# jaak-s/BayesianDataFusion.jl

Measured on AMD Instinct MI355X. Metric: Gibbs sweeps/sec (both entities) + test RMSE, MovieLens-1M D=32, higher is better.
Workload: dtype f64; 1 GPU; BPMF MovieLens-1M 6040x3952, 500209 training ratings (500000 held out), D=32, alpha=1.5, step = rows of both entities + hyperpriors + test prediction update (one native call); BEFORE the --warmup steps the engine's set-up runs 60 ms of full iterations whose results are discarded (device_warmup_ms); num_latent=32, burnin=5, psamples=1985, parallelism=1 GPU

## Files before the change

bayesiandatafusion.jl_amd/csrc/k_rows_col.hip:

```cpp
#include "rows.h"
#include "dpp_rows32.h"
#include <algorithm>

#ifndef BDF_COL_WAVES
#define BDF_COL_WAVES 2
#endif
#define COL_PSZ 800

#ifdef BDF_K1_STAMPS
#define CSTAMP_DECL unsigned long long st_t = __builtin_amdgcn_s_memtime(), st_acc = 0, st_mid = 0, st_prior = 0, st_fin = 0, st_rng = 0, st_steps = 0, st_rounds = 0, st_parts = 0, st_fins = 0, st_folds = 0; const unsigned long long st_begin = st_t
#define CSTAMP(x) do { const unsigned long long now_ = __builtin_amdgcn_s_memtime(); x += now_ - st_t; st_t = now_; } while (0)
#else
#define CSTAMP_DECL do { } while (0)
#define CSTAMP(x) do { } while (0)
#endif

namespace {

template <int DR, int K>
__device__ __forceinline__ void col_obs(double (&A0)[33], double (&A1)[33], double v0, double v1, double r)
{
    col_rank1<DR, 0>(A0, A1, v0, v1);
    fm1_run<K>(A0[32], r, v0);
    fm1_run<K>(A1[32], r, v1);
}

__device__ __forceinline__ double col_ld(__amdgpu_buffer_rsrc_t rs, uint32_t off)
{
    typedef unsigned u2v __attribute__((ext_vector_type(2)));
    const u2v x = __builtin_amdgcn_raw_buffer_load_b64(rs, (int)off, 0, 0);
    return __hiloint2double((int)x.y, (int)x.x);
}

template <bool FULL, int K0>
__device__ __forceinline__ void col_gather4(double (&b)[4][2], __amdgpu_buffer_rsrc_t rs, uint32_t idw, uint32_t rowb, uint32_t eo, bool ok1)
{
#pragma unroll
    for (int q = 0; q < 4; q++) {
        uint32_t id;
        if (q == 0) id = row_bcast_u32<K0>(idw); else if (q == 1) id = row_bcast_u32<K0 + 1>(idw);
        else if (q == 2) id = row_bcast_u32<K0 + 2>(idw); else id = row_bcast_u32<K0 + 3>(idw);
        if constexpr (FULL) {
            const uint32_t base = id + eo;
            b[q][1] = col_ld(rs, base);
            b[q][0] = col_ld(rs, base + 128u);
        } else {
            const uint32_t base = id + eo;
            b[q][0] = col_ld(rs, base);
            b[q][1] = col_ld(rs, ok1 ? base - 128u : 0xffffffffu);
        }
    }
}
template <int DR, int K0>
__device__ __forceinline__ void col_compute4(double (&A0)[33], double (&A1)[33], const double (&b)[4][2], double r)
{
    col_obs<DR, K0>(A0, A1, b[0][0], b[0][1], r);
    col_obs<DR, K0 + 1>(A0, A1, b[1][0], b[1][1], r);
    col_obs<DR, K0 + 2>(A0, A1, b[2][0], b[2][1], r);
    col_obs<DR, K0 + 3>(A0, A1, b[3][0], b[3][1], r);
}

template <int X>
__device__ __forceinline__ void col_fold(double (&A0)[33], double (&A1)[33], double m)
{
#pragma unroll
    for (int i = 0; i < 33; i++) A0[i] = fma(__shfl_xor(A0[i], X), m, A0[i]);
#pragma unroll
    for (int i = 16; i < 33; i++) A1[i] = fma(__shfl_xor(A1[i], X), m, A1[i]);
}

template <int E0, int E1, bool ADD>
__device__ __forceinline__ void col_slot_load(double (&A0)[33], double (&A1)[33], const double *src, double m)
{
#pragma unroll
    for (int e = E0; e < E1; e++) {
        const double v = src[e * 16];
        double &d = e < 33 ? A0[e] : A1[e - 17];
        if (ADD) d = fma(v, m, d); else d = v * m;
    }
}

__device__ __forceinline__ void col_prior_dma(const double *image, unsigned lds_dst, int lane)
{
    const void *sbase = (const void *)(((uint64_t)(uint32_t)__builtin_amdgcn_readfirstlane((int)((uint64_t)image >> 32)) << 32) |
                                       (uint32_t)__builtin_amdgcn_readfirstlane((int)(uint32_t)(uint64_t)image));
#pragma unroll
    for (int k = 0; k < 6; k++) {
        const unsigned voff = (unsigned)k * 1024u + (unsigned)lane * 16u;
        unsigned keep;
        asm volatile("s_mov_b32 %0, m0\n\ts_mov_b32 m0, %2\n\ts_nop 0\n\tglobal_load_lds_dwordx4 %1, %3 sc1\n\ts_mov_b32 m0, %0"
                     : "=&s"(keep) : "v"(voff), "s"(lds_dst + (unsigned)k * 1024u), "s"(sbase) : "memory");
    }
}
template <int S, int I, int DR>
__device__ __forceinline__ void col_prior_lds(double (&A)[33], const double *img, double alpha, int j)
{
    if constexpr (I < DR) {
        A[I] = fma(alpha, A[I], img[sys_off<S, I>(j)]);
        col_prior_lds<S, I + 1, DR>(A, img, alpha, j);
    }
}

template <int DR, bool FULL>
__global__ __launch_bounds__(64, BDF_COL_WAVES) void k_rows_col(SampleArgs a_in, ColPlanDev p_in, uint32_t fac_bytes)
{
    __shared__ __attribute__((aligned(16))) double lds[4 * 272 + 768];
    const int w = blockIdx.x;
    if (w >= p_in.n_waves) return;
    const int r_end = p_in.wave_round[w + 1];
    if (a_in.span && threadIdx.x == 0) atomicMin(a_in.span + 2 * (w & 63), (unsigned long long)__builtin_amdgcn_s_memrealtime());
    CSTAMP_DECL;
#pragma nounroll
    for (int rd = p_in.wave_round[w]; rd < r_end; rd++) {
    int zero = 0, lane = threadIdx.x;
    asm volatile("" : "+s"(zero), "+v"(lane));
    const SampleArgs &a = (&a_in)[zero];
    const ColPlanDev &p = (&p_in)[zero];
    const int j = lane & 15, g = lane >> 4;
    const TermDev &T = a.t[0];
    const int D = FULL ? 32 : a.D;
    const int ec0 = D - 1 - j, ec1 = D - 17 - j;
    const int n0 = ec0, n1 = ec1 >= 0 ? ec1 : 0;
    const bool ok1 = ec1 >= 0;
    const uint32_t rowb = (uint32_t)D * 8u;
    const uint32_t eo = FULL ? (uint32_t)ec1 * 8u : (uint32_t)ec0 * 8u;
    const __amdgpu_buffer_rsrc_t rs = __builtin_amdgcn_make_buffer_rsrc((void *)T.fac[0], 0, (int)fac_bytes, 0x00020000);
    const bool coded = T.packed != nullptr;
    const double mean = T.mean;
    {
        const ColJob jb = p.jobs[(int64_t)rd * 4 + g];
        const bool live = jb.row >= 0;
        const int n = live ? jb.count : 0;
        const unsigned lds_img = (unsigned)__builtin_amdgcn_readfirstlane((int)(unsigned)(size_t)(__attribute__((address_space(3))) double *)(lds + 4 * 272));
        bool have_prior = true;
        if (a.ready) have_prior = __builtin_amdgcn_readfirstlane((int)((int32_t)(__hip_atomic_load(a.ready, __ATOMIC_RELAXED, __HIP_MEMORY_SCOPE_AGENT) - a.ready_want) >= 0)) != 0;
        if (have_prior) col_prior_dma(a.prior_c, lds_img, lane);
        double A0[33], A1[33];
#pragma unroll
        for (int i = 0; i < 33; i++) { A0[i] = 0.0; A1[i] = 0.0; }
        int nmax = n;
        nmax = max(nmax, __shfl_xor(nmax, 16));
        nmax = max(nmax, __shfl_xor(nmax, 32));
        nmax = __builtin_amdgcn_readfirstlane(nmax);
        if (nmax > 0) {
            const uint32_t *packed = coded ? T.packed + jb.q_begin : nullptr;
            const int32_t *colidx = T.colidx + jb.q_begin;
            const double *vals = T.vals + jb.q_begin;
            const double *table = T.table;
#define COL_CHUNK(c0, IDW, R)                                                                     \
            {                                                                                     \
                const int o_ = (c0) + j;                                                          \
                IDW = 0xffffffu; R = 0.0;                                                         \
                if (o_ < n) {                                                                     \
                    if (coded) { const uint32_t pw_ = packed[o_]; IDW = pw_; R = table[pw_ >> 24] - mean; } \
                    else { IDW = (uint32_t)colidx[o_]; R = vals[o_] - mean; }                     \
                }                                                                                 \
                IDW = __umul24(IDW, rowb);       \
            }
            uint32_t idw_c, idw_n;
            double r_c, r_n;
            COL_CHUNK(0, idw_c, r_c)
            double ba[4][2], bb[4][2];
            col_gather4<FULL, 0>(ba, rs, idw_c, rowb, eo, ok1);
            for (int c0 = 0;; c0 += 16) {
                COL_CHUNK(c0 + 16, idw_n, r_n)
                col_gather4<FULL, 4>(bb, rs, idw_c, rowb, eo, ok1);
                __builtin_amdgcn_sched_barrier(0);
                col_compute4<DR, 0>(A0, A1, ba, r_c);
                if (c0 + 4 >= nmax) break;
                col_gather4<FULL, 8>(ba, rs, idw_c, rowb, eo, ok1);
                __builtin_amdgcn_sched_barrier(0);
                col_compute4<DR, 4>(A0, A1, bb, r_c);
                if (c0 + 8 >= nmax) break;
                col_gather4<FULL, 12>(bb, rs, idw_c, rowb, eo, ok1);
                __builtin_amdgcn_sched_barrier(0);
                col_compute4<DR, 8>(A0, A1, ba, r_c);
                if (c0 + 12 >= nmax) break;
                col_gather4<FULL, 0>(ba, rs, idw_n, rowb, eo, ok1);
                __builtin_amdgcn_sched_barrier(0);
                col_compute4<DR, 12>(A0, A1, bb, r_c);
                if (c0 + 16 >= nmax) break;
                idw_c = idw_n; r_c = r_n;
            }
#undef COL_CHUNK
        }
#ifdef BDF_K1_STAMPS
        asm volatile("s_nop 0" :: "v"(A0[0]), "v"(A0[32]), "v"(A1[31]));
        st_steps += (unsigned long long)nmax; st_rounds++;
#endif
        CSTAMP(st_acc);
        const unsigned fl = (unsigned)jb.flags;
        if (__builtin_amdgcn_readfirstlane((int)(__ballot((fl & COLF_PAIR) != 0) != 0ull))) {
#ifdef BDF_K1_STAMPS
            st_folds++;
#endif
            col_fold<16>(A0, A1, (fl & COLF_PAIR) ? 1.0 : 0.0);
            if (__builtin_amdgcn_readfirstlane((int)(__ballot((fl & COLF_QUAD) != 0) != 0ull)))
                col_fold<32>(A0, A1, (fl & COLF_QUAD) ? 1.0 : 0.0);
        }
        if (__builtin_amdgcn_readfirstlane((int)(fl & COLF_MULTI))) {
            const int srow = __builtin_amdgcn_readfirstlane(jb.srow);
            double *dst = p.partials + (int64_t)__builtin_amdgcn_readfirstlane(jb.slot) * COL_PSZ + j;
            if (g == 0) {
#pragma unroll
                for (int e = 0; e < 33; e++) __hip_atomic_store(dst + e * 16, A0[e], __ATOMIC_RELAXED, __HIP_MEMORY_SCOPE_AGENT);
#pragma unroll
                for (int e = 33; e < 50; e++) __hip_atomic_store(dst + e * 16, A1[e - 17], __ATOMIC_RELAXED, __HIP_MEMORY_SCOPE_AGENT);
            }
            const ColSplit sr = p.rows[srow];
            asm volatile("s_waitcnt vmcnt(0)" ::: "memory");
            int old = 0;
            if (lane == 0) old = __hip_atomic_fetch_add(p.arrived + srow, 1, __ATOMIC_RELAXED, __HIP_MEMORY_SCOPE_AGENT);
            old = __builtin_amdgcn_readfirstlane(old);
#ifdef BDF_K1_STAMPS
            st_parts++;
            if (old == sr.n_slots - 1) st_fins++;
#endif
            if (old != sr.n_slots - 1) { CSTAMP(st_mid); continue; }
            __builtin_amdgcn_fence(__ATOMIC_ACQUIRE, "agent");
            asm volatile("s_waitcnt vmcnt(0)" ::: "memory");
            if (lane == 0) p.arrived[srow] = 0;
            const double *src = p.partials + (int64_t)sr.slot_begin * COL_PSZ + j;
            col_slot_load<0, 50, false>(A0, A1, src + (int64_t)(g < sr.n_slots ? g : 0) * COL_PSZ, g < sr.n_slots ? 1.0 : 0.0);
            for (int s0 = 4; s0 < sr.n_slots; s0 += 4) {
                const bool on = s0 + g < sr.n_slots;
                const double *sp = src + (int64_t)(on ? s0 + g : 0) * COL_PSZ;
                const double m = on ? 1.0 : 0.0;
                col_slot_load<0, 16, true>(A0, A1, sp, m);
                asm volatile("" ::: "memory");
                col_slot_load<16, 33, true>(A0, A1, sp, m);
                asm volatile("" ::: "memory");
                col_slot_load<33, 50, true>(A0, A1, sp, m);
                asm volatile("" ::: "memory");
            }
            col_fold<16>(A0, A1, 1.0);
            col_fold<32>(A0, A1, 1.0);
        }
        CSTAMP(st_mid);
        double z0 = 0.0, z1 = 0.0;
        {
            double ze = 0.0, zo = 0.0;
            if (live && 2 * j < D) bdf_normal_pair(a.seed, a.sweep, BDF_P_ROW, a.entity_tag, (uint64_t)(uint32_t)jb.orig, (uint32_t)j, ze, zo);
            const int base = lane & 48;
            const double ze0 = __shfl(ze, base + (n0 >> 1)), zo0 = __shfl(zo, base + (n0 >> 1));
            const double ze1 = __shfl(ze, base + (n1 >> 1)), zo1 = __shfl(zo, base + (n1 >> 1));
            z0 = (n0 & 1) ? zo0 : ze0;
            z1 = ok1 ? ((n1 & 1) ? zo1 : ze1) : 0.0;
        }
        asm volatile("" ::: "memory");
        CSTAMP(st_rng);
        {
            double *tl = lds + g * 272;
#pragma unroll
            for (int r = 0; r < 16; r++) tl[r * 17 + j] = A0[16 + r];
            wave_sync();
#pragma unroll
            for (int i = 0; i < 16; i++) A1[i] = tl[j * 17 + i];
            wave_sync();
        }
        CSTAMP(st_mid);
        const double alpha = term_alpha(T);
        if (!have_prior) {
            int spins = 0;
            while ((int32_t)(__hip_atomic_load(a.ready, __ATOMIC_RELAXED, __HIP_MEMORY_SCOPE_AGENT) - a.ready_want) < 0) {
                __builtin_amdgcn_s_sleep(16);
                if (++spins > (1 << 22)) { if (lane == 0) atomicOr_system(a.flag, 16); break; }
            }
            col_prior_dma(a.prior_c, lds_img, lane);
        }
        {
            const double *pb = a.prior_b + (a.mu_is_matrix && live ? (int64_t)jb.row * D : 0);
            const double b0 = __hip_atomic_load(pb + n0, __ATOMIC_RELAXED, __HIP_MEMORY_SCOPE_AGENT);
            const double b1 = __hip_atomic_load(pb + n1, __ATOMIC_RELAXED, __HIP_MEMORY_SCOPE_AGENT);
            asm volatile("s_waitcnt vmcnt(0)" ::: "memory");
            wave_sync();
            const double *img = lds + 4 * 272;
            col_prior_lds<0, 0, DR>(A0, img, alpha, j);
            col_prior_lds<1, 0, DR>(A1, img, alpha, j);
            A0[32] = fma(alpha, A0[32], b0);
            A1[32] = ok1 ? fma(alpha, A1[32], b1) : 0.0;
            wave_sync();
        }
#ifdef BDF_K1_STAMPS
        asm volatile("s_nop 0" :: "v"(A0[0]), "v"(A0[31]), "v"(A1[0]), "v"(A1[31]));
#endif
        CSTAMP(st_prior);
        double d0 = 1.0, d1 = 1.0;
        fin_factor<DR, 0>(A0, A1, d0, d1, j);
        const bool lead = live && (fl & COLF_LEADER);
        if (lead && (!(d0 > 0.0) || (ok1 && !(d1 > 0.0)))) atomicOr_system(a.flag, 1);
        const double rd0 = fast_rcp(d0), rd1 = fast_rcp(d1);
        double y0 = fma(z0, fast_rsqrt(d0), A0[32] * rd0), y1 = fma(z1, fast_rsqrt(d1), A1[32] * rd1);
        fin_backward<DR - 1>(A0, A1, y0, y1, rd0, rd1, j);
        if (lead) __hip_atomic_store(a.out + ((int64_t)jb.row * D + ec0), y0, __ATOMIC_RELAXED, __HIP_MEMORY_SCOPE_AGENT);
        if (lead && ok1) __hip_atomic_store(a.out + ((int64_t)jb.row * D + ec1), y1, __ATOMIC_RELAXED, __HIP_MEMORY_SCOPE_AGENT);
        CSTAMP(st_fin);
    }
    }
    if (a_in.done) {
        asm volatile("s_waitcnt vmcnt(0)" ::: "memory");
        if (threadIdx.x == 0) __hip_atomic_fetch_add(a_in.done + BDF_DONE_STRIDE * (w & (BDF_DONE_SHARDS - 1)), 1u, __ATOMIC_RELAXED, __HIP_MEMORY_SCOPE_AGENT);
    }
    if (a_in.span && threadIdx.x == 0) atomicMax(a_in.span + 2 * (w & 63) + 1, (unsigned long long)__builtin_amdgcn_s_memrealtime());
#ifdef BDF_K1_STAMPS
    if (threadIdx.x == 0 && a_in.b_dump && w < 65536) {
        unsigned long long *d = (unsigned long long *)a_in.b_dump + (size_t)w * 16;
        d[0] = st_begin; d[8] = st_t; d[6] = st_rounds; d[7] = st_steps;
        d[1] = st_parts; d[2] = st_fins; d[3] = st_folds;
        d[11] = st_rng; d[12] = st_acc; d[13] = st_mid; d[14] = st_prior; d[15] = st_fin;
        d[9] = __builtin_amdgcn_s_getreg((4 - 1) << 11 | 0 << 6 | 4) | ((unsigned long long)__builtin_amdgcn_s_getreg((32 - 1) << 11 | 0 << 6 | 4));
        d[10] = __builtin_amdgcn_s_getreg((4 - 1) << 11 | 0 << 6 | 20);
    }
#endif
}

#define COL_C_OBS 56.0
#define COL_C_FIN 1460.0
#define COL_C_FOLD 180.0
#define COL_C_PART 700.0

struct Round { ColJob job[4]; double cost; };

ColJob idle_job() { return ColJob{-1, 0, 0, 0, -1, 0, 0}; }

}

int bdf_col_plan_build(bdf_ctx *ctx, const std::vector<bdf_row_ref> &rows, int T, int64_t slots, bdf_col_plan &plan)
{
    std::vector<Round> rounds;
    std::vector<ColSplit> splits;
    struct Unit { int32_t row, orig; int64_t qb; int32_t n; };
    std::vector<Unit> singles, pairs;
    int32_t n_slots_total = 0;
    auto quad_round = [&](const bdf_row_ref &rr, int64_t b0, int64_t b1, int32_t srow, int32_t slot, double fin_share) {
        Round R;
        const int64_t m = b1 - b0;
        int32_t lmax = 0;
        for (int q = 0; q < 4; q++) {
            const int64_t p0 = b0 + m * q / 4, p1 = b0 + m * (q + 1) / 4;
            R.job[q] = ColJob{rr.out, rr.orig, rr.qb + p0, (int32_t)(p1 - p0), srow, slot,
                              (int32_t)(COLF_PAIR | COLF_QUAD | (q == 0 ? COLF_LEADER : 0) | (srow >= 0 ? COLF_MULTI : 0))};
            lmax = std::max(lmax, (int32_t)(p1 - p0));
        }
        constexpr double part_extra = 3000.0;
        R.cost = COL_C_OBS * lmax + 2 * COL_C_FOLD + (srow >= 0 ? COL_C_PART + fin_share + part_extra : COL_C_FIN);
        rounds.push_back(R);
    };
    for (const bdf_row_ref &rr : rows) {
        const int64_t n = rr.cnt;
        if (n <= T) singles.push_back(Unit{rr.out, rr.orig, rr.qb, (int32_t)n});
        else if (n <= 2 * (int64_t)T) pairs.push_back(Unit{rr.out, rr.orig, rr.qb, (int32_t)n});
        else if (n <= 4 * (int64_t)T) quad_round(rr, 0, n, -1, 0, 0.0);
        else {
            const int64_t W = (n + 4 * (int64_t)T - 1) / (4 * (int64_t)T);
            BDF_REQUIRE(W < (1 << 20), BDF_ERR_ARG, "bdf_sample_rows: a row of %lld observations", (long long)n);
            const int32_t srow = (int32_t)splits.size();
            splits.push_back(ColSplit{n_slots_total, (int32_t)W});
            const double share = (COL_C_FIN + 2 * COL_C_FOLD + 60.0 * (double)((W + 3) / 4)) / (double)W;
            for (int64_t q = 0; q < W; q++) quad_round(rr, n * q / W, n * (q + 1) / W, srow, n_slots_total + (int32_t)q, share);
            n_slots_total += (int32_t)W;
        }
    }
    auto by_len = [](const Unit &x, const Unit &y) { return x.n > y.n; };
    std::stable_sort(pairs.begin(), pairs.end(), by_len);
    std::stable_sort(singles.begin(), singles.end(), by_len);
    auto pair_jobs = [](const Unit &u, ColJob *dst) {
        const int32_t h = u.n / 2;
        dst[0] = ColJob{u.row, u.orig, u.qb, h, -1, 0, COLF_PAIR | COLF_LEADER};
        dst[1] = ColJob{u.row, u.orig, u.qb + h, u.n - h, -1, 0, COLF_PAIR};
    };
    size_t si = 0;
    for (size_t pi = 0; pi < pairs.size(); pi += 2) {
        Round R;
        pair_jobs(pairs[pi], R.job);
        int32_t lmax = pairs[pi].n - pairs[pi].n / 2;
        if (pi + 1 < pairs.size()) pair_jobs(pairs[pi + 1], R.job + 2);
        else {
            for (int q = 2; q < 4; q++) {
                if (si < singles.size()) {
                    const Unit &u = singles[si++];
                    R.job[q] = ColJob{u.row, u.orig, u.qb, u.n, -1, 0, COLF_LEADER};
                    lmax = std::max(lmax, u.n);
                } else R.job[q] = idle_job();
            }
        }
        R.cost = COL_C_OBS * lmax + COL_C_FOLD + COL_C_FIN;
        rounds.push_back(R);
    }
    for (; si < singles.size(); si += 4) {
        Round R;
        for (int q = 0; q < 4; q++) {
            if (si + q < singles.size()) {
                const Unit &u = singles[si + q];
                R.job[q] = ColJob{u.row, u.orig, u.qb, u.n, -1, 0, COLF_LEADER};
            } else R.job[q] = idle_job();
        }
        R.cost = COL_C_OBS * singles[si].n + COL_C_FIN;
        rounds.push_back(R);
    }
    plan.n_rounds = (int64_t)rounds.size();
    plan.n_waves = 0;
    plan.n_split_rows = (int32_t)splits.size();
    if (rounds.empty()) return BDF_OK;
    (void)slots;
    const int64_t nw = (int64_t)rounds.size();
    std::vector<int32_t> rank(rounds.size());
    for (size_t i = 0; i < rank.size(); i++) rank[i] = (int32_t)i;
    std::stable_sort(rank.begin(), rank.end(), [&](int32_t x, int32_t y) { return rounds[(size_t)x].cost > rounds[(size_t)y].cost; });
    constexpr int64_t S2 = 896;
    std::vector<int32_t> idx;
    idx.reserve(rounds.size());
    if (nw <= S2) idx = rank;
    else {
        const int64_t two = std::min<int64_t>(nw, 2 * S2);
        const int64_t P = two - S2, A = S2 - P;
        for (int64_t i = 0; i < P; i++) idx.push_back(rank[(size_t)(A + i)]);
        for (int64_t i = 0; i < A; i++) idx.push_back(rank[(size_t)i]);
        for (int64_t i = 0; i < P; i++) idx.push_back(rank[(size_t)(two - 1 - i)]);
        for (int64_t i = two; i < nw; i++) idx.push_back(rank[(size_t)i]);
    }
    std::vector<ColJob> jobs;
    std::vector<int32_t> wave_round;
    jobs.reserve(rounds.size() * 4);
    wave_round.push_back(0);
    for (int32_t i : idx) {
        for (int q = 0; q < 4; q++) jobs.push_back(rounds[(size_t)i].job[q]);
        wave_round.push_back((int32_t)(jobs.size() / 4));
    }
    plan.cost_max = rounds[(size_t)rank.front()].cost;
    plan.cost_min = rounds[(size_t)rank.back()].cost;
    plan.n_waves = (int32_t)nw;
    BDF_HIP(hipMalloc((void **)&plan.jobs_dev, jobs.size() * sizeof(ColJob)));
    BDF_HIP(hipMemcpy(plan.jobs_dev, jobs.data(), jobs.size() * sizeof(ColJob), hipMemcpyHostToDevice));
    BDF_HIP(hipMalloc((void **)&plan.wave_round_dev, wave_round.size() * sizeof(int32_t)));
    BDF_HIP(hipMemcpy(plan.wave_round_dev, wave_round.data(), wave_round.size() * sizeof(int32_t), hipMemcpyHostToDevice));
    BDF_HIP(hipMalloc((void **)&plan.rows_dev, std::max<size_t>(splits.size() * sizeof(ColSplit), 8)));
    if (!splits.empty()) BDF_HIP(hipMemcpy(plan.rows_dev, splits.data(), splits.size() * sizeof(ColSplit), hipMemcpyHostToDevice));
    BDF_HIP(hipMalloc((void **)&plan.partials_dev, std::max<size_t>((size_t)n_slots_total * COL_PSZ * sizeof(double), 8)));
    BDF_HIP(hipMalloc((void **)&plan.arrived_dev, std::max<size_t>(splits.size() * sizeof(int32_t), 8)));
    BDF_HIP(hipMemsetAsync(plan.arrived_dev, 0, std::max<size_t>(splits.size() * sizeof(int32_t), 8), ctx->stream));
    return BDF_OK;
}

void bdf_col_plan_free(bdf_col_plan &plan)
{
    if (plan.jobs_dev) (void)hipFree(plan.jobs_dev);
    if (plan.wave_round_dev) (void)hipFree(plan.wave_round_dev);
    if (plan.rows_dev) (void)hipFree(plan.rows_dev);
    if (plan.partials_dev) (void)hipFree(plan.partials_dev);
    if (plan.arrived_dev) (void)hipFree(plan.arrived_dev);
    plan = bdf_col_plan{};
}

int bdf_col_launch(bdf_ctx *ctx, const SampleArgs &a, const bdf_col_plan &plan, int64_t M_other, hipEvent_t e0, hipEvent_t e1)
{
    if (plan.n_waves <= 0) return BDF_OK;
    ColPlanDev p;
    p.jobs = plan.jobs_dev; p.wave_round = plan.wave_round_dev; p.n_waves = plan.n_waves; p._pad = 0;
    p.rows = plan.rows_dev; p.partials = plan.partials_dev; p.arrived = plan.arrived_dev;
    const int64_t bytes = M_other * (int64_t)a.D * 8;
    BDF_REQUIRE(bytes < ((int64_t)1 << 32), BDF_ERR_ARG, "bdf_sample_rows: the column kernel needs a factor matrix below 4 GiB");
    const uint32_t fb = (uint32_t)bytes;
    const dim3 grid((unsigned)plan.n_waves), block(64);
    const int DR = (a.D + 3) / 4 * 4;
#define COL_LAUNCH(DRV, FULLV) hipExtLaunchKernelGGL((k_rows_col<DRV, FULLV>), grid, block, 0, ctx->stream, e0, e1, 0, a, p, fb)
    if (a.D == 32) COL_LAUNCH(32, true);
    else if (DR <= 20) COL_LAUNCH(20, false);
    else if (DR <= 24) COL_LAUNCH(24, false);
    else if (DR <= 28) COL_LAUNCH(28, false);
    else COL_LAUNCH(32, false);
#undef COL_LAUNCH
    BDF_HIP(hipGetLastError());
    return BDF_OK;
}
```

Before: 12630 sweeps/s.

## Overlap normal RNG with first gather and DMA prior mean into LDS

```diff
diff --git a/bayesiandatafusion.jl_amd/csrc/k_rows_col.hip b/bayesiandatafusion.jl_amd/csrc/k_rows_col.hip
--- a/bayesiandatafusion.jl_amd/csrc/k_rows_col.hip
+++ b/bayesiandatafusion.jl_amd/csrc/k_rows_col.hip
@@ -8,7 +8,7 @@
 #define COL_PSZ 800
 
 #ifdef BDF_K1_STAMPS
-#define CSTAMP_DECL unsigned long long st_t = __builtin_amdgcn_s_memtime(), st_acc = 0, st_mid = 0, st_prior = 0, st_fin = 0, st_rng = 0, st_steps = 0, st_rounds = 0, st_parts = 0, st_fins = 0, st_folds = 0; const unsigned long long st_begin = st_t
+#define CSTAMP_DECL unsigned long long st_t = __builtin_amdgcn_s_memtime(), st_acc = 0, st_mid = 0, st_prior = 0, st_fin = 0, st_rng = 0, st_head = 0, st_erng = 0, st_steps = 0, st_rounds = 0, st_parts = 0, st_fins = 0, st_folds = 0; const unsigned long long st_begin = st_t
 #define CSTAMP(x) do { const unsigned long long now_ = __builtin_amdgcn_s_memtime(); x += now_ - st_t; st_t = now_; } while (0)
 #else
 #define CSTAMP_DECL do { } while (0)
@@ -92,6 +92,35 @@
                      : "=&s"(keep) : "v"(voff), "s"(lds_dst + (unsigned)k * 1024u), "s"(sbase) : "memory");
     }
 }
+__device__ __forceinline__ void col_mean_dma(const double *src, int D, bool matrix, unsigned lds_dst, int lane)
+{
+    const uint32_t *row = (const uint32_t *)src;
+    if (!matrix) {
+        const uint32_t *gp = row + (lane < 2 * D ? lane : 0);
+        unsigned keep;
+        asm volatile("s_mov_b32 %0, m0\n\ts_mov_b32 m0, %2\n\ts_nop 0\n\tglobal_load_lds_dword %1, off sc1\n\ts_mov_b32 m0, %0"
+                     : "=&s"(keep) : "v"(gp), "s"(lds_dst) : "memory");
+    } else {
+#pragma unroll
+        for (int k = 0; k < 4; k++) {
+            const int d = k * 16 + (lane & 15);
+            const uint32_t *gp = row + (d < 2 * D ? d : 0);
+            unsigned keep;
+            asm volatile("s_mov_b32 %0, m0\n\ts_mov_b32 m0, %2\n\ts_nop 0\n\tglobal_load_lds_dword %1, off sc1\n\ts_mov_b32 m0, %0"
+                         : "=&s"(keep) : "v"(gp), "s"(lds_dst + (unsigned)k * 256u) : "memory");
+        }
+    }
+}
+__device__ __forceinline__ int col_mean_at(int n, int g, bool matrix) { return matrix ? (n >> 3) * 32 + g * 8 + (n & 7) : n; }
+
+__device__ __forceinline__ void col_normals_park(double *park, const SampleArgs &a, bool live, int D, int32_t orig, int j)
+{
+    double ze = 0.0, zo = 0.0;
+    if (live && 2 * j < D) bdf_normal_pair(a.seed, a.sweep, BDF_P_ROW, a.entity_tag, (uint64_t)(uint32_t)orig, (uint32_t)j, ze, zo);
+    park[2 * j] = ze;
+    park[2 * j + 1] = zo;
+}
+
 template <int S, int I, int DR>
 __device__ __forceinline__ void col_prior_lds(double (&A)[33], const double *img, double alpha, int j)
 {
@@ -104,7 +133,7 @@
 template <int DR, bool FULL>
 __global__ __launch_bounds__(64, BDF_COL_WAVES) void k_rows_col(SampleArgs a_in, ColPlanDev p_in, uint32_t fac_bytes)
 {
-    __shared__ __attribute__((aligned(16))) double lds[4 * 272 + 768];
+    __shared__ __attribute__((aligned(16))) double lds[4 * 272 + 768 + 128];
     const int w = blockIdx.x;
     if (w >= p_in.n_waves) return;
     const int r_end = p_in.wave_round[w + 1];
@@ -134,7 +163,14 @@
         const unsigned lds_img = (unsigned)__builtin_amdgcn_readfirstlane((int)(unsigned)(size_t)(__attribute__((address_space(3))) double *)(lds + 4 * 272));
         bool have_prior = true;
         if (a.ready) have_prior = __builtin_amdgcn_readfirstlane((int)((int32_t)(__hip_atomic_load(a.ready, __ATOMIC_RELAXED, __HIP_MEMORY_SCOPE_AGENT) - a.ready_want) >= 0)) != 0;
-        if (have_prior) col_prior_dma(a.prior_c, lds_img, lane);
+        const bool mu_rows = a.mu_is_matrix != 0;
+        if (have_prior) {
+            col_prior_dma(a.prior_c, lds_img, lane);
+            col_mean_dma(a.prior_b + (mu_rows && live ? (int64_t)jb.row * D : 0), D, mu_rows, lds_img + 768u * 8u, lane);
+        }
+        const unsigned fl = (unsigned)jb.flags;
+        const bool early = __builtin_amdgcn_readfirstlane((int)(fl & COLF_MULTI)) == 0;
+        double *park = lds + g * 32;
         double A0[33], A1[33];
 #pragma unroll
         for (int i = 0; i < 33; i++) { A0[i] = 0.0; A1[i] = 0.0; }
@@ -142,7 +178,7 @@
         nmax = max(nmax, __shfl_xor(nmax, 16));
         nmax = max(nmax, __shfl_xor(nmax, 32));
         nmax = __builtin_amdgcn_readfirstlane(nmax);
-        if (nmax > 0) {
+        {
             const uint32_t *packed = coded ? T.packed + jb.q_begin : nullptr;
             const int32_t *colidx = T.colidx + jb.q_begin;
             const double *vals = T.vals + jb.q_begin;
@@ -157,12 +193,21 @@
                 }                                                                                 \
                 IDW = __umul24(IDW, rowb);       \
             }
-            uint32_t idw_c, idw_n;
-            double r_c, r_n;
-            COL_CHUNK(0, idw_c, r_c)
-            double ba[4][2], bb[4][2];
-            col_gather4<FULL, 0>(ba, rs, idw_c, rowb, eo, ok1);
-            for (int c0 = 0;; c0 += 16) {
+            uint32_t idw_c = 0, idw_n;
+            double r_c = 0.0, r_n;
+            double ba[4][2] = {}, bb[4][2];
+            if (nmax > 0) {
+                COL_CHUNK(0, idw_c, r_c)
+                col_gather4<FULL, 0>(ba, rs, idw_c, rowb, eo, ok1);
+            }
+            asm volatile("" ::: "memory");
+            __builtin_amdgcn_sched_barrier(0);
+            CSTAMP(st_head);
+            if (early) col_normals_park(park, a, live, D, jb.orig, j);
+            asm volatile("" ::: "memory");
+            __builtin_amdgcn_sched_barrier(0);
+            CSTAMP(st_erng);
+            if (nmax > 0) for (int c0 = 0;; c0 += 16) {
                 COL_CHUNK(c0 + 16, idw_n, r_n)
                 col_gather4<FULL, 4>(bb, rs, idw_c, rowb, eo, ok1);
                 __builtin_amdgcn_sched_barrier(0);
@@ -189,7 +234,6 @@
         st_steps += (unsigned long long)nmax; st_rounds++;
 #endif
         CSTAMP(st_acc);
-        const unsigned fl = (unsigned)jb.flags;
         if (__builtin_amdgcn_readfirstlane((int)(__ballot((fl & COLF_PAIR) != 0) != 0ull))) {
 #ifdef BDF_K1_STAMPS
             st_folds++;
@@ -198,7 +242,7 @@
             if (__builtin_amdgcn_readfirstlane((int)(__ballot((fl & COLF_QUAD) != 0) != 0ull)))
                 col_fold<32>(A0, A1, (fl & COLF_QUAD) ? 1.0 : 0.0);
         }
-        if (__builtin_amdgcn_readfirstlane((int)(fl & COLF_MULTI))) {
+        if (!early) {
             const int srow = __builtin_amdgcn_readfirstlane(jb.srow);
             double *dst = p.partials + (int64_t)__builtin_amdgcn_readfirstlane(jb.slot) * COL_PSZ + j;
             if (g == 0) {
@@ -217,6 +261,11 @@
             if (old == sr.n_slots - 1) st_fins++;
 #endif
             if (old != sr.n_slots - 1) { CSTAMP(st_mid); continue; }
+            CSTAMP(st_mid);
+            col_normals_park(park, a, live, D, jb.orig, j);
+            asm volatile("" ::: "memory");
+            __builtin_amdgcn_sched_barrier(0);
+            CSTAMP(st_rng);
             __builtin_amdgcn_fence(__ATOMIC_ACQUIRE, "agent");
             asm volatile("s_waitcnt vmcnt(0)" ::: "memory");
             if (lane == 0) p.arrived[srow] = 0;
@@ -237,17 +286,9 @@
             col_fold<32>(A0, A1, 1.0);
         }
         CSTAMP(st_mid);
-        double z0 = 0.0, z1 = 0.0;
-        {
-            double ze = 0.0, zo = 0.0;
-            if (live && 2 * j < D) bdf_normal_pair(a.seed, a.sweep, BDF_P_ROW, a.entity_tag, (uint64_t)(uint32_t)jb.orig, (uint32_t)j, ze, zo);
-            const int base = lane & 48;
-            const double ze0 = __shfl(ze, base + (n0 >> 1)), zo0 = __shfl(zo, base + (n0 >> 1));
-            const double ze1 = __shfl(ze, base + (n1 >> 1)), zo1 = __shfl(zo, base + (n1 >> 1));
-            z0 = (n0 & 1) ? zo0 : ze0;
-            z1 = ok1 ? ((n1 & 1) ? zo1 : ze1) : 0.0;
-        }
-        asm volatile("" ::: "memory");
+        wave_sync();
+        const double z0 = park[n0], z1 = ok1 ? park[n1] : 0.0;
+        wave_sync();
         CSTAMP(st_rng);
         {
             double *tl = lds + g * 272;
@@ -269,12 +310,20 @@
             col_prior_dma(a.prior_c, lds_img, lane);
         }
         {
-            const double *pb = a.prior_b + (a.mu_is_matrix && live ? (int64_t)jb.row * D : 0);
-            const double b0 = __hip_atomic_load(pb + n0, __ATOMIC_RELAXED, __HIP_MEMORY_SCOPE_AGENT);
-            const double b1 = __hip_atomic_load(pb + n1, __ATOMIC_RELAXED, __HIP_MEMORY_SCOPE_AGENT);
+            double b0 = 0.0, b1 = 0.0;
+            if (!have_prior) {
+                const double *pb = a.prior_b + (mu_rows && live ? (int64_t)jb.row * D : 0);
+                b0 = __hip_atomic_load(pb + n0, __ATOMIC_RELAXED, __HIP_MEMORY_SCOPE_AGENT);
+                b1 = __hip_atomic_load(pb + n1, __ATOMIC_RELAXED, __HIP_MEMORY_SCOPE_AGENT);
+            }
             asm volatile("s_waitcnt vmcnt(0)" ::: "memory");
             wave_sync();
             const double *img = lds + 4 * 272;
+            if (have_prior) {
+                const double *pbl = img + 768;
+                b0 = pbl[col_mean_at(n0, g, mu_rows)];
+                b1 = pbl[col_mean_at(n1, g, mu_rows)];
+            }
             col_prior_lds<0, 0, DR>(A0, img, alpha, j);
             col_prior_lds<1, 0, DR>(A1, img, alpha, j);
             A0[32] = fma(alpha, A0[32], b0);
@@ -307,6 +356,7 @@
         unsigned long long *d = (unsigned long long *)a_in.b_dump + (size_t)w * 16;
         d[0] = st_begin; d[8] = st_t; d[6] = st_rounds; d[7] = st_steps;
         d[1] = st_parts; d[2] = st_fins; d[3] = st_folds;
+        d[4] = st_head; d[5] = st_erng;
         d[11] = st_rng; d[12] = st_acc; d[13] = st_mid; d[14] = st_prior; d[15] = st_fin;
         d[9] = __builtin_amdgcn_s_getreg((4 - 1) << 11 | 0 << 6 | 4) | ((unsigned long long)__builtin_amdgcn_s_getreg((32 - 1) << 11 | 0 << 6 | 4));
         d[10] = __builtin_amdgcn_s_getreg((4 - 1) << 11 | 0 << 6 | 20);
```

After: 12720 sweeps/s (median of 6 runs). About the same (+0.7%).
